# YunjiKim/Unsupervised-Keypoint-Learning-for-Guiding-Class-conditional-Video-Prediction

Hardware: AMD Instinct MI355X
Metric: detector_translator train frames/sec @128x128 K=15 (higher is better)
Workload: dtype f32

## Files before the change

profiles/step_breakdown.py:

```python
#!/usr/bin/env python3
import csv
import sys

FAMILIES = [
    ('bf16-storage 3x3 conv fwd/dgrad (conv3x3_bf16s)', ('conv3x3_bf16s_kernel',)),
    ('bf16 3x3 weight gradient (conv3x3_wgrad_bf16 + slab reduce)', ('conv3x3_wgrad_bf16_kernel', 'wgrad16_reduce_kernel')),
    ('bf16 filter preparation', ('conv_bf16s_prepare',)),
    ('bf16 <-> fp32 conversions / bf16 channel copies', ('cast_channels_kernel',)),
    ('F(4x4,3x3) Winograd fwd/dgrad, bf16x3 form (conv_wino43b)', ('conv_wino43b_kernel',)),
    ('F(4x4,3x3) Winograd fwd/dgrad, fp32 MFMA (conv_wino43)', ('conv_wino43_kernel',)),
    ('F(2x2,3x3) Winograd fwd/dgrad', ('conv_wino_v2_kernel',)),
    ('Winograd weight gradient', ('conv_wino_wgrad_kernel',)),
    ('bf16x3 gather conv fwd/dgrad (conv_gemm3)', ('conv_gemm3_kernel',)),
    ('bf16x3 weight gradient (conv_wgrad3)', ('conv_wgrad3_kernel',)),
    ('fp32-MFMA direct conv fwd/dgrad', ('conv_igemm_kernel', 'conv_small_cout_kernel')),
    ('fp32-MFMA direct weight gradients', ('conv_wgrad_kernel', 'conv_wgrad_rows', 'conv_wgrad_tap_rows', 'conv_wgrad_rows_merged', 'conv_c16_wgrad', 'wgrad_small')),
    ('split-K / weight-gradient slab reductions', ('wgrad_reduce_kernel', 'splitk_reduce_kernel')),
    ('16-cout / image-input conv kernels', ('conv3x3_c16_kernel', 'conv_rgb', 'conv_few')),
    ('batch norm', ('bn_', 'chan_reduce_kernel<1', 'chan_reduce_kernel<2', 'chan_reduce_bf16_kernel<1', 'chan_reduce_bf16_kernel<2')),
    ('bias gradients (channel sums)', ('chan_reduce_kernel<0', 'chan_reduce_bf16_kernel<0', 'chan_sum_finalize')),
    ('Winograd filter transforms', ('filter_transform',)),
    ('key-point head / heat-map render', ('kp_', 'gauss_')),
    ('VGG19 pointwise (prep, pool, feature gradient, L1)', ('vgg_', 'maxpool2', 'l1_pair')),
    ('resize / concat / copy / activation backward / blend', ('resize2x', 'copy_channels', 'act_bwd', 'head_blend', 'fill_kernel', 'axpy')),
    ('Adam', ('adam_tf',)),
    ('losses', ('xent',)),
    ('torch glue (adds, mean)', ('at::native',)),
]


def main():
    path, steps = sys.argv[1], float(sys.argv[2])
    rows = list(csv.DictReader(open(path)))
    fam = {name: [0.0, 0] for name, _ in FAMILIES}
    other = [0.0, 0, []]
    for r in rows:
        ns, calls = float(r['TotalDurationNs']), int(r['Calls'])
        for name, keys in FAMILIES:
            if any(k in r['Name'] for k in keys):
                fam[name][0] += ns; fam[name][1] += calls
                break
        else:
            other[0] += ns; other[1] += calls; other[2].append(r['Name'][:50])
    total = sum(v[0] for v in fam.values()) + other[0]
    launches = sum(v[1] for v in fam.values()) + other[1]
    print('%-58s %9s %10s' % ('kernel family', 'ms/step', 'launches/step'))
    for name, _ in FAMILIES:
        ns, calls = fam[name]
        if calls:
            print('%-58s %9.3f %10.1f' % (name, ns / 1e6 / steps, calls / steps))
    if other[1]:
        print('%-58s %9.3f %10.1f   %s' % ('other', other[0] / 1e6 / steps, other[1] / steps, sorted(set(other[2]))[:6]))
    print('%-58s %9.3f %10.1f   (sum over the three streams)' % ('TOTAL', total / 1e6 / steps, launches / steps))


if __name__ == '__main__':
    main()
```

unsupervised-keypoint-learning-for-guiding-class-conditional-video-prediction_amd/csrc/conv_wino.hip:

```cpp
#include "kpx_internal.h"
#include "kpx_env.h"
#include <stdlib.h>
#include <type_traits>
#include <atomic>

struct WinoGeom {
    const float* x; float* y; const float* U; const float* bias;
    int N, H, W, Cin, ldx, Cout, ldy, act;
    int pack;
    int Kp, Np;
    int tiles_y, tiles_x, nt;
    int stagger;
    float* stats;
    const float* mask_y; int ld_mask;
    const float* bn_beta;
};

static __device__ __attribute__((aligned(16))) float wino_zero16[4] = {0.f, 0.f, 0.f, 0.f};

template <bool DGRAD>
__global__ __launch_bounds__(256) void wino_filter_transform_frag_kernel(const float* __restrict__ w, int Cin, int Cout, int Kp, int Np, float* __restrict__ Uf) {
    const int K = DGRAD ? Cout : Cin, Nn = DGRAD ? Cin : Cout;
    const int KC = Kp >> 3, NB = Np >> 5;
    const size_t total = (size_t)Kp * Np;
    for (size_t idx = (size_t)blockIdx.x * 256 + threadIdx.x; idx < total; idx += (size_t)gridDim.x * 256) {
        const int j = (int)(idx & 3), li = (int)((idx >> 2) & 31), lh = (int)((idx >> 7) & 1);
        const size_t blk = idx >> 8;
        const int nb = (int)(blk % NB), kc = (int)(blk / NB);
        const int c = 8 * kc + 4 * lh + j, n = 32 * nb + li;
        const bool real = c < K && n < Nn;
        float g[3][3];
#pragma unroll
        for (int r = 0; r < 3; ++r)
#pragma unroll
            for (int q = 0; q < 3; ++q)
                g[r][q] = !real ? 0.f : (DGRAD ? w[((size_t)((2 - r) * 3 + (2 - q)) * Cin + n) * Cout + c] : w[((size_t)(r * 3 + q) * Cin + c) * Cout + n]);
        float t[4][3];
#pragma unroll
        for (int q = 0; q < 3; ++q) {
            t[0][q] = g[0][q];
            t[1][q] = 0.5f * (g[0][q] + g[1][q] + g[2][q]);
            t[2][q] = 0.5f * (g[0][q] - g[1][q] + g[2][q]);
            t[3][q] = g[2][q];
        }
        const size_t pstride = (size_t)KC * NB * 256;
        float* o = Uf + blk * 256 + (idx & 255);
#pragma unroll
        for (int i = 0; i < 4; ++i) {
            o[(size_t)(i * 4 + 0) * pstride] = t[i][0];
            o[(size_t)(i * 4 + 1) * pstride] = 0.5f * (t[i][0] + t[i][1] + t[i][2]);
            o[(size_t)(i * 4 + 2) * pstride] = 0.5f * (t[i][0] - t[i][1] + t[i][2]);
            o[(size_t)(i * 4 + 3) * pstride] = t[i][2];
        }
    }
}

__device__ __forceinline__ int w8_pos(int p) { return p < 8 ? p : (p == 16 ? 8 : (p == 17 ? 17 : p + 1)); }
__device__ __forceinline__ int w8_pix(int pos) { return pos < 8 ? pos : (pos == 8 ? 16 : (pos == 17 ? 17 : pos - 1)); }

#define W2_RAW 3200
#define W2_V 8192
#define W2_MAIN (2 * W2_RAW + 2 * W2_V)

#ifdef KPX_WINO_STAMP
__device__ unsigned long long* wino_dbg = nullptr;
extern "C" int kpx_debug_wino_stamps(unsigned long long* buf) { return -(int)hipMemcpyToSymbol(HIP_SYMBOL(wino_dbg), &buf, sizeof(buf)); }
#define W2_STAMP(slot) do { if (dbg) dbg[(slot)] = __builtin_amdgcn_s_memtime(); } while (0)
#else
#define W2_STAMP(slot) do { } while (0)
#endif

template <int MODE, int STATS>
__global__ __launch_bounds__(512, 2) void conv_wino_v2_kernel(const WinoGeom g) {
    extern __shared__ __attribute__((aligned(16))) float smem[];
    constexpr int NC = 32 * MODE, NTG = MODE;
    float* const rawb = smem;
    float* const Vb = smem + 2 * W2_RAW;

    const int t = threadIdx.x, lane = t & 63, wave = t >> 6;
    const int li = lane & 31, lh = lane >> 5;
    const int wa = wave & 3, hsel = wave >> 2;
    int L = kpx_xcd_remap(blockIdx.x, gridDim.x);
    const int ntc = g.Np / NC;
    const int nti = L % ntc; L /= ntc;
    const int bx = L % g.tiles_x; L /= g.tiles_x;
    const int by = L % g.tiles_y;
    const int n = g.pack ? 4 * L : L / g.tiles_y;
    const int oy0 = by * 16, ox0 = bx * 16, n0 = nti * NC;

    const float* rp[2]; bool rok[2];
#pragma unroll
    for (int i = 0; i < 2; ++i) {
        const int u = t + 512 * i, q = u >> 1, py = q / 20, ps = q - py * 20;
        int iy, ix, ni = n;
        bool ok;
        if (g.pack) {
            const int sy = py / 10, sx = ps / 10;
            iy = py - 10 * sy - 1; ix = ps - 10 * sx - 1; ni = n + 2 * sy + sx;
            ok = u < 800 && (unsigned)iy < 8u && (unsigned)ix < 8u;
        } else {
            iy = oy0 - 1 + py; ix = ox0 - 1 + w8_pix(ps);
            ok = u < 720 && ps < 18 && (unsigned)iy < (unsigned)g.H && (unsigned)ix < (unsigned)g.W;
        }
        if (g.Cin <= 4 && (u & 1)) ok = false;
        rok[i] = ok;
        rp[i] = ok ? g.x + ((size_t)(ni * g.H + iy) * g.W + ix) * g.ldx + (u & 1) * 4 : wino_zero16;
    }
    const int KC = g.Kp >> 3, NB = g.Np >> 5;
    const int nb = MODE == 2 ? nti * 2 + hsel : nti;
    const size_t ub_pstride = (size_t)KC * NB * 256, ub_step = (size_t)NB * 256;
    const float* ubp = g.U + ((size_t)(4 * wa) * KC * NB + nb) * 256 + lane * 4;
    const int tslot = t & 1, ttile = (t >> 1) & 63, vrow = t >> 7;
    const int tty = ttile >> 3, ttx = ttile & 7;
    const int ra = vrow == 0 ? 0 : (vrow == 2 ? 2 : 1), rb = vrow == 0 ? 2 : (vrow == 1 ? 2 : (vrow == 2 ? 1 : 3));
    const float sgn = vrow == 1 ? 1.f : -1.f;
    int trd[4];
#pragma unroll
    for (int c = 0; c < 4; ++c)
        trd[c] = g.pack ? ((tty >> 2) * 10 + 2 * (tty & 3) + ra) * 160 + ((ttx >> 2) * 10 + 2 * (ttx & 3) + c) * 8 + tslot * 4
                        : (2 * tty + ra) * 160 + w8_pos(2 * ttx + c) * 8 + tslot * 4;
    const int trb = (rb - ra) * 160;
    const int vwr = (vrow * 4) * 512 + ttile * 8 + ((tslot ^ ((ttile >> 3) & 1)) << 2);
    int a_rd[NTG];
#pragma unroll
    for (int i = 0; i < NTG; ++i) {
        const int tile = (MODE == 2 ? i : hsel) * 32 + li;
        a_rd[i] = (4 * wa) * 512 + tile * 8 + ((lh ^ ((tile >> 3) & 1)) << 2);
    }

    f32x16 acc[4][NTG];
#pragma unroll
    for (int b = 0; b < 4; ++b)
#pragma unroll
        for (int i = 0; i < NTG; ++i)
#pragma unroll
            for (int r = 0; r < 16; ++r) acc[b][i][r] = 0.f;

    const int nchunks = g.Kp / 8;
    const int ktail = g.Cin - (nchunks - 1) * 8 - tslot * 4;
    f32x4 rr[2], ub[4];
    auto load_raw = [&]() {
#pragma unroll
        for (int i = 0; i < 2; ++i) { rr[i] = *reinterpret_cast<const f32x4*>(rp[i]); if (rok[i]) rp[i] += 8; }
    };
    const int st2 = t < 288 ? (t + 512) * 4 : t * 4;
    auto stage = [&](float* rawW) {
        *reinterpret_cast<f32x4*>(&rawW[t * 4]) = rr[0];
        *reinterpret_cast<f32x4*>(&rawW[st2]) = t < 288 ? rr[1] : rr[0];
    };
    auto transform = [&](const float* rawR, float* Vw, bool mask_tail) {
        f32x4 tr[4];
#pragma unroll
        for (int c = 0; c < 4; ++c) {
            const f32x4 a = *reinterpret_cast<const f32x4*>(&rawR[trd[c]]);
            const f32x4 b = *reinterpret_cast<const f32x4*>(&rawR[trd[c] + trb]);
            tr[c] = a + sgn * b;
        }
        if (mask_tail) {
#pragma unroll
            for (int c = 0; c < 4; ++c)
#pragma unroll
                for (int j = 0; j < 4; ++j) if (j >= ktail) tr[c][j] = 0.f;
        }
        *reinterpret_cast<f32x4*>(&Vw[vwr]) = tr[0] - tr[2];
        *reinterpret_cast<f32x4*>(&Vw[vwr + 512]) = tr[1] + tr[2];
        *reinterpret_cast<f32x4*>(&Vw[vwr + 1024]) = tr[2] - tr[1];
        *reinterpret_cast<f32x4*>(&Vw[vwr + 1536]) = tr[1] - tr[3];
    };
    auto mfma = [&](const float* Vr, bool refill) {
        f32x4 av[2][NTG];
#pragma unroll
        for (int i = 0; i < NTG; ++i) av[0][i] = *reinterpret_cast<const f32x4*>(&Vr[a_rd[i]]);
#pragma unroll
        for (int b = 0; b < 4; ++b) {
            if (b < 3) {
#pragma unroll
                for (int i = 0; i < NTG; ++i) av[(b + 1) & 1][i] = *reinterpret_cast<const f32x4*>(&Vr[a_rd[i] + (b + 1) * 512]);
            }
#pragma unroll
            for (int j = 0; j < 4; ++j)
#pragma unroll
                for (int i = 0; i < NTG; ++i)
                    acc[b][i] = __builtin_amdgcn_mfma_f32_32x32x2f32(av[b & 1][i][j], ub[b][j], acc[b][i], 0, 0, 0);
            if (refill) ub[b] = *reinterpret_cast<const f32x4*>(ubp + (size_t)b * ub_pstride);
        }
        ubp += ub_step;
    };
    const bool late = g.stagger && __builtin_amdgcn_readfirstlane(t) >= 256;
#ifdef KPX_WINO_STAMP
    unsigned long long* dbg = (wino_dbg && lane == 0 && (wave & 3) == 0 && blockIdx.x < 64) ? wino_dbg + ((size_t)blockIdx.x * 2 + (wave >> 2)) * 256 : nullptr;
    if (dbg) { dbg[0] = __builtin_amdgcn_s_memtime(); dbg[1] = __builtin_amdgcn_s_memrealtime(); }
#endif
    auto body = [&](int k, auto full_tag, auto parity_tag) {
        constexpr bool FULL = decltype(full_tag)::value;
        constexpr int PAR = decltype(parity_tag)::value;
        const int cur = PAR == 2 ? (k & 1) : PAR;
        float* const rawC = rawb + cur * W2_RAW;
        float* const rawN = rawb + (cur ^ 1) * W2_RAW;
        float* const Vc = Vb + cur * W2_V;
        float* const Vn = Vb + (cur ^ 1) * W2_V;
        W2_STAMP(8 + 4 * k);
        __syncthreads();
        W2_STAMP(9 + 4 * k);
        if (late) mfma(Vc, FULL || k + 1 < nchunks);
        if (late) W2_STAMP(10 + 4 * k);
        if (FULL || k + 1 < nchunks) transform(rawN, Vn, !FULL && k + 1 == nchunks - 1 && ktail < 4);
        if (FULL || k + 2 < nchunks) stage(rawC);
        if (FULL || k + 3 < nchunks) load_raw();
        if (!late) W2_STAMP(10 + 4 * k);
        if (!late) mfma(Vc, FULL || k + 1 < nchunks);
        W2_STAMP(11 + 4 * k);
    };

    load_raw();
#pragma unroll
    for (int b = 0; b < 4; ++b) ub[b] = *reinterpret_cast<const f32x4*>(ubp + (size_t)b * ub_pstride);
    ubp += ub_step;
    stage(rawb);
    if (nchunks > 1) load_raw();
    __syncthreads();
    transform(rawb, Vb, nchunks == 1 && ktail < 4);
    if (nchunks > 1) stage(rawb + W2_RAW);
    if (nchunks > 2) load_raw();
    int k = 0;
    for (; k + 4 < nchunks; k += 2) {
        body(k, std::true_type{}, std::integral_constant<int, 0>{});
        body(k + 1, std::true_type{}, std::integral_constant<int, 1>{});
    }
    for (; k < nchunks; ++k) body(k, std::false_type{}, std::integral_constant<int, 2>{});

#ifdef KPX_WINO_STAMP
    if (dbg) { dbg[2] = __builtin_amdgcn_s_memtime(); }
#endif
    __syncthreads();
    float* const P = smem;
#pragma unroll
    for (int i = 0; i < NTG; ++i) {
        const int tg = MODE == 2 ? i : hsel;
#pragma unroll
        for (int r = 0; r < 16; ++r) {
            const float m0 = acc[0][i][r], m1 = acc[1][i][r], m2 = acc[2][i][r], m3 = acc[3][i][r];
            const int tile = tg * 32 + (r & 3) + 8 * (r >> 2) + 4 * lh;
            const int col = (MODE == 2 ? hsel * 32 : 0) + li;
            P[((wa * 2 + 0) * 64 + tile) * NC + col] = m0 + m1 + m2;
            P[((wa * 2 + 1) * 64 + tile) * NC + col] = m1 - m2 - m3;
        }
    }
    const bool mask_vec = STATS == 2 && (g.ld_mask & 3) == 0 && ((reinterpret_cast<uintptr_t>(g.mask_y) & 15) == 0);
    f32x4 ym[MODE][4];
    if (STATS == 2) {
#pragma unroll
        for (int it = 0; it < MODE; ++it) {
            const int idx = t + 512 * it;
            const int tile = idx / (NC / 4), cq = idx - tile * (NC / 4), c0 = n0 + cq * 4;
            const int oy = oy0 + 2 * (tile >> 3), ox = ox0 + 2 * (tile & 7);
#pragma unroll
            for (int px = 0; px < 4; ++px) {
                const float* my = g.mask_y + ((size_t)(n * g.H + oy + (px >> 1)) * g.W + ox + (px & 1)) * g.ld_mask + c0;
                ym[it][px] = f32x4{0.f, 0.f, 0.f, 0.f};
                if (mask_vec && c0 + 3 < g.Cout) ym[it][px] = *reinterpret_cast<const f32x4*>(my);
                else {
#pragma unroll
                    for (int e = 0; e < 4; ++e) if (c0 + e < g.Cout) ym[it][px][e] = my[e];
                }
            }
        }
    }
    __syncthreads();
    const bool vec_ok = (g.ldy & 3) == 0 && ((reinterpret_cast<uintptr_t>(g.y) & 15) == 0);
    f32x4 st_s = {0.f, 0.f, 0.f, 0.f}, st_q = {0.f, 0.f, 0.f, 0.f};
#pragma unroll
    for (int it = 0; it < MODE; ++it) {
        const int idx = t + 512 * it;
        const int tile = idx / (NC / 4), cq = idx - tile * (NC / 4);
        f32x4 pv[4][2];
#pragma unroll
        for (int a = 0; a < 4; ++a)
#pragma unroll
            for (int j = 0; j < 2; ++j) pv[a][j] = *reinterpret_cast<const f32x4*>(&P[((a * 2 + j) * 64 + tile) * NC + cq * 4]);
        const int c0 = n0 + cq * 4;
        f32x4 bv = {0.f, 0.f, 0.f, 0.f};
        if (g.bias) {
#pragma unroll
            for (int e = 0; e < 4; ++e) if (c0 + e < g.Cout) bv[e] = g.bias[c0 + e];
        }
        f32x4 bvec = {0.f, 0.f, 0.f, 0.f};
        if (STATS == 2) {
#pragma unroll
            for (int e = 0; e < 4; ++e) if (c0 + e < g.Cout) bvec[e] = g.bn_beta[c0 + e];
        }
        const int ty = tile >> 3, tx = tile & 7;
        const int on = g.pack ? n + 2 * (ty >> 2) + (tx >> 2) : n;
        const int oy = g.pack ? 2 * (ty & 3) : oy0 + 2 * ty, ox = g.pack ? 2 * (tx & 3) : ox0 + 2 * tx;
#pragma unroll
        for (int dy = 0; dy < 2; ++dy)
#pragma unroll
            for (int dx = 0; dx < 2; ++dx) {
                f32x4 v = (dy == 0 ? pv[0][dx] + pv[1][dx] + pv[2][dx] : pv[1][dx] - pv[2][dx] - pv[3][dx]) + bv;
                if (g.act == KPX_ACT_RELU) {
#pragma unroll
                    for (int e = 0; e < 4; ++e) v[e] = fmaxf(v[e], 0.f);
                } else if (g.act == KPX_ACT_LRELU) {
#pragma unroll
                    for (int e = 0; e < 4; ++e) v[e] = v[e] > 0.f ? v[e] : 0.01f * v[e];
                }
                if (STATS == 2) {
                    const f32x4 yv = ym[it][dy * 2 + dx];
#pragma unroll
                    for (int e = 0; e < 4; ++e) {
                        const float dz = yv[e] > 0.f ? v[e] : 0.f;
                        st_s[e] += dz; st_q[e] += dz * (yv[e] - bvec[e]);
                    }
                } else if (STATS == 1) { st_s += v; st_q += v * v; }
                float* o = g.y + ((size_t)(on * g.H + oy + dy) * g.W + ox + dx) * g.ldy + c0;
                if (vec_ok && c0 + 3 < g.Cout) *reinterpret_cast<f32x4*>(o) = v;
                else {
#pragma unroll
                    for (int e = 0; e < 4; ++e) if (c0 + e < g.Cout) o[e] = v[e];
                }
            }
    }
    if (STATS != 0) {
        __syncthreads();
        float* const S = smem;
        *reinterpret_cast<f32x4*>(&S[t * 8]) = st_s;
        *reinterpret_cast<f32x4*>(&S[t * 8 + 4]) = st_q;
        __syncthreads();
        if (t < 2 * NC) {
            const int stat = t / NC, c = t - stat * NC, cq = c >> 2, e = c & 3;
            float r = 0.f;
#pragma unroll 8
            for (int m = 0; m < 512 / (NC / 4); ++m) r += S[(cq + (NC / 4) * m) * 8 + stat * 4 + e];
            const size_t tile_id = ((size_t)n * g.tiles_y + by) * g.tiles_x + bx;
            if (n0 + c < g.Cout) g.stats[(tile_id * 2 + stat) * g.Cout + n0 + c] = r;
        }
    }
#ifdef KPX_WINO_STAMP
    if (dbg) { dbg[3] = __builtin_amdgcn_s_memtime(); dbg[4] = __builtin_amdgcn_s_memrealtime(); }
#endif
}

static inline int w2_lds_bytes(int mode) { const int main = W2_MAIN * 4, epi = 4 * 2 * 64 * 32 * mode * 4; return main > epi ? main : epi; }

static std::atomic<unsigned long long> wino_attr_mask{0};

extern "C" int kpx_conv3x3_wino_eligible(int N, int H, int W, int K, int Nn, int ldin, const void* in_ptr) {
    if (kpx_env()->no_wino || N <= 0 || K <= 0 || Nn <= 0) return 0;
    const bool shape = (H % 16 == 0 && W % 16 == 0) || (H == 8 && W == 8 && N % 4 == 0);
    const int kmin = 4, nmin = 4;
    const bool kfit = ldin >= ((K + 7) & ~7) || K == 4;
    return shape && K >= kmin && Nn >= nmin && (K >= 16 || K == 4 || K == 8) && kfit && (ldin % 4 == 0) && (((uintptr_t)in_ptr) & 15) == 0;
}
extern "C" __attribute__((visibility("hidden"))) int kpx_wino_eligible(int N, int H, int W, int K, int Nn, int ldin, const void* in_ptr) {
    return kpx_conv3x3_wino_eligible(N, H, W, K, Nn, ldin, in_ptr);
}

extern "C" size_t kpx_wino_u_bytes(int Cin, int Cout) {
    const size_t a = (size_t)((Cin + 7) & ~7) * ((Cout + 31) & ~31), b = (size_t)((Cout + 7) & ~7) * ((Cin + 31) & ~31);
    return 16 * 4 * (a > b ? a : b);
}

extern "C" int kpx_wino_filter_transform_f32(const float* w_hwio, int Cin, int Cout, int dgrad, float* U, void* stream) {
    if (!w_hwio || !U || Cin <= 0 || Cout <= 0) return KPX_EINVAL;
    const int K = dgrad ? Cout : Cin, Nn = dgrad ? Cin : Cout;
    const int Kp = (K + 7) & ~7, Np = (Nn + 31) & ~31;
    const size_t pairs = (size_t)Kp * Np;
    size_t nb = (pairs + 255) / 256; if (nb > 1024) nb = 1024;
    hipStream_t s = kpx_stream(stream);
    if (dgrad) hipLaunchKernelGGL(wino_filter_transform_frag_kernel<true>, dim3((unsigned)nb), dim3(256), 0, s, w_hwio, Cin, Cout, Kp, Np, U);
    else hipLaunchKernelGGL(wino_filter_transform_frag_kernel<false>, dim3((unsigned)nb), dim3(256), 0, s, w_hwio, Cin, Cout, Kp, Np, U);
    return kpx_launch_status();
}

__global__ __launch_bounds__(256) void wino_filter_transform_batch_kernel(const KpxWinoDesc* __restrict__ descs) {
    const KpxWinoDesc d = descs[blockIdx.y];
    const int Cin = d.cin, Cout = d.cout;
    const bool dg = d.dgrad != 0;
    const int K = dg ? Cout : Cin, Nn = dg ? Cin : Cout;
    const int Kp = (K + 7) & ~7, Np = (Nn + 31) & ~31, KC = Kp >> 3, NB = Np >> 5;
    const size_t total = (size_t)Kp * Np, pstride = (size_t)KC * NB * 256;
    const float* __restrict__ w = d.w;
    float* __restrict__ Uf = d.u;
    for (size_t idx = (size_t)blockIdx.x * 256 + threadIdx.x; idx < total; idx += (size_t)gridDim.x * 256) {
        const int j = (int)(idx & 3), li = (int)((idx >> 2) & 31), lh = (int)((idx >> 7) & 1);
        const size_t blk = idx >> 8;
        const int nb = (int)(blk % NB), kc = (int)(blk / NB);
        const int c = 8 * kc + 4 * lh + j, n = 32 * nb + li;
        const bool real = c < K && n < Nn;
        float g[3][3];
#pragma unroll
        for (int r = 0; r < 3; ++r)
#pragma unroll
            for (int q = 0; q < 3; ++q)
                g[r][q] = !real ? 0.f : (dg ? w[((size_t)((2 - r) * 3 + (2 - q)) * Cin + n) * Cout + c] : w[((size_t)(r * 3 + q) * Cin + c) * Cout + n]);
        float t[4][3];
#pragma unroll
        for (int q = 0; q < 3; ++q) {
            t[0][q] = g[0][q];
            t[1][q] = 0.5f * (g[0][q] + g[1][q] + g[2][q]);
            t[2][q] = 0.5f * (g[0][q] - g[1][q] + g[2][q]);
            t[3][q] = g[2][q];
        }
        float* o = Uf + blk * 256 + (idx & 255);
#pragma unroll
        for (int i = 0; i < 4; ++i) {
            o[(size_t)(i * 4 + 0) * pstride] = t[i][0];
            o[(size_t)(i * 4 + 1) * pstride] = 0.5f * (t[i][0] + t[i][1] + t[i][2]);
            o[(size_t)(i * 4 + 2) * pstride] = 0.5f * (t[i][0] - t[i][1] + t[i][2]);
            o[(size_t)(i * 4 + 3) * pstride] = t[i][2];
        }
    }
}
extern "C" int kpx_wino_filter_transform_batch_f32(const void* descs_dev, int n, void* stream) {
    if (!descs_dev || n <= 0 || n > 65535) return KPX_EINVAL;
    hipLaunchKernelGGL(wino_filter_transform_batch_kernel, dim3(64, (unsigned)n), dim3(256), 0, kpx_stream(stream), (const KpxWinoDesc*)descs_dev);
    return kpx_launch_status();
}

extern "C" size_t kpx_conv3x3_wino_stats_tiles(int N, int H, int W) {
    return (H % 16 || W % 16 || N <= 0) ? 0 : (size_t)N * (H / 16) * (W / 16);
}
static int wino_launch(const float* in, int N, int H, int W, int K, int ldin, const float* U, const float* bias,
                       float* out, int Nn, int ldout, int act, float* tile_stats, void* stream,
                       const float* mask_y, int ld_mask, const float* bn_beta) {
    if (!in || !U || !out || ldin < (K == 4 ? 4 : K) || ldout < Nn || act < 0 || act > 2 || !kpx_conv3x3_wino_eligible(N, H, W, K, Nn, ldin, in)) return KPX_EINVAL;
    hipStream_t s = kpx_stream(stream);
    if (kpx_first_use_on_device(&wino_attr_mask)) {
        hipError_t e = hipSuccess;
#define W2_ATTR(M, S) if (e == hipSuccess) e = hipFuncSetAttribute(reinterpret_cast<const void*>(conv_wino_v2_kernel<M, S>), hipFuncAttributeMaxDynamicSharedMemorySize, w2_lds_bytes(M))
        W2_ATTR(1, 0); W2_ATTR(2, 0); W2_ATTR(1, 1); W2_ATTR(2, 1); W2_ATTR(1, 2); W2_ATTR(2, 2);
#undef W2_ATTR
        if (e != hipSuccess) return -(int)e;
    }
    WinoGeom g{};
    g.x = in; g.y = out; g.U = U; g.bias = bias; g.stats = tile_stats;
    g.mask_y = mask_y; g.ld_mask = ld_mask; g.bn_beta = bn_beta;
    g.N = N; g.H = H; g.W = W; g.Cin = K; g.ldx = ldin; g.Cout = Nn; g.ldy = ldout; g.act = act;
    g.Kp = (K + 7) & ~7; g.Np = (Nn + 31) & ~31;
    g.pack = (H == 8 && W == 8) ? 1 : 0;
    g.tiles_y = g.pack ? 1 : H / 16; g.tiles_x = g.pack ? 1 : W / 16; g.nt = g.Np / 32;
    const unsigned blocks = (unsigned)((size_t)(g.pack ? N / 4 : N) * g.tiles_y * g.tiles_x * g.nt);
    const bool wide = blocks / 2 >= 256 && g.Np % 64 == 0;
    g.stagger = 1;
    const int st = !tile_stats ? 0 : (mask_y ? 2 : 1);
#define W2_GO(M, S) hipLaunchKernelGGL((conv_wino_v2_kernel<M, S>), dim3(M == 2 ? blocks / 2 : blocks), dim3(512), w2_lds_bytes(M), s, g)
    if (wide) { if (st == 0) W2_GO(2, 0); else if (st == 1) W2_GO(2, 1); else W2_GO(2, 2); }
    else { if (st == 0) W2_GO(1, 0); else if (st == 1) W2_GO(1, 1); else W2_GO(1, 2); }
#undef W2_GO
    return kpx_launch_status();
}

extern "C" int kpx_conv3x3_wino_f32(const float* in, int N, int H, int W, int K, int ldin, const float* U, const float* bias,
                                    float* out, int Nn, int ldout, int act, float* tile_stats, const float* bn_y, int ld_bn_y,
                                    const float* bn_beta, void* stream) {
    if (tile_stats && (H % 16 || W % 16)) return KPX_EINVAL;
    if ((bn_y || bn_beta) && (!tile_stats || !bn_y || !bn_beta || ld_bn_y < Nn || bias || act != KPX_ACT_NONE)) return KPX_EINVAL;
    return wino_launch(in, N, H, W, K, ldin, U, bias, out, Nn, ldout, act, tile_stats, stream, bn_y, ld_bn_y, bn_beta);
}

extern "C" __attribute__((visibility("hidden"))) int kpx_wino_conv3x3(const float* in, int N, int H, int W, int K, int ldin, const float* w_hwio, int Cin, int Cout, int dgrad,
                                const float* bias, int act, float* out, int Nn, int ldout, float* U_ws, hipStream_t s) {
    int rc = kpx_wino_filter_transform_f32(w_hwio, Cin, Cout, dgrad, U_ws, (void*)s);
    if (rc) return rc;
    return kpx_conv3x3_wino_f32(in, N, H, W, K, ldin, U_ws, bias, out, Nn, ldout, act, nullptr, nullptr, 0, nullptr, (void*)s);
}

struct WinoWgradGeom {
    const float* x; const float* dy; float* out;
    int N, H, W, Cin, ldx, Cout, lddy;
    int cit, cot, S, cps, total_chunks, chy, chx;
    size_t slab;
};

template <int CIT, int COT>
__global__ __launch_bounds__(512, 2) void conv_wino_wgrad_kernel(const WinoWgradGeom g) {
    constexpr int CI = 32 * CIT, CO = 32 * COT, SI = CI / 4, SO = CO / 4;
    constexpr int VF = 16 * 8 * CI, DF = 16 * 8 * CO, BUF = VF + DF;
    extern __shared__ __attribute__((aligned(16))) float smem[];

    const int t = threadIdx.x, lane = t & 63, wave = __builtin_amdgcn_readfirstlane(t >> 6), li = lane & 31, lh = lane >> 5;
    int L = kpx_xcd_remap(blockIdx.x, gridDim.x);
    const int split = L % g.S; L /= g.S;
    const int cot = L % g.cot, cit = L / g.cot;
    const int c0 = cit * CI, n0 = cot * CO;

    const int vsl = (t % SI) * 4, vtile = (t / SI) & 7, vrow = t / (8 * SI);
    const int esl = (t % SO) * 4, etile = (t / SO) & 7, erow = t / (8 * SO);
    const bool vthr = t < 32 * SI, ethr = t < 32 * SO;
    const bool vact = vthr && c0 + vsl < g.Cin, eact = ethr && n0 + esl < g.Cout;
    const int xtail = g.Cin - (c0 + vsl);
    const int ra = vrow == 0 ? 0 : (vrow == 2 ? 2 : 1), rb = vrow == 0 ? 2 : (vrow == 1 ? 2 : (vrow == 2 ? 1 : 3));
    const float sgn = vrow == 1 ? 1.f : -1.f;
    const int pya = 2 * (vtile >> 2) + ra - 1, pyb = 2 * (vtile >> 2) + rb - 1, px0 = 2 * (vtile & 3) - 1;
    const int vwr = (vrow * 4) * 8 * CI + vtile * CI + vsl;
    const float d0 = erow == 3 ? 0.f : 1.f, d1 = erow == 0 ? 0.f : (erow == 1 ? 1.f : -1.f);
    const int dwr = VF + (erow * 4) * 8 * CO + etile * CO + esl;
    const int dyo = ((2 * (etile >> 2) * g.W + 2 * (etile & 3)) * g.lddy + n0 + esl) * 4;
    const int OOB = (int)0x80000000;
    const __amdgpu_buffer_rsrc_t rsx = __builtin_amdgcn_make_buffer_rsrc(const_cast<float*>(g.x) - (size_t)(g.W + 1) * g.ldx, 0, 0x7fffffff, 0x00020000);
    const __amdgpu_buffer_rsrc_t rsd = __builtin_amdgcn_make_buffer_rsrc(const_cast<float*>(g.dy), 0, 0x7fffffff, 0x00020000);
    int vxa[4], vxb[4], vd[4];
#pragma unroll
    for (int c = 0; c < 4; ++c) {
        vxa[c] = vact ? (((pya + 1) * g.W + px0 + c + 1) * g.ldx + c0 + vsl) * 4 : OOB;
        vxb[c] = vact ? (((pyb + 1) * g.W + px0 + c + 1) * g.ldx + c0 + vsl) * 4 : OOB;
    }
    vd[0] = eact ? dyo : OOB; vd[1] = eact ? dyo + g.lddy * 4 : OOB; vd[2] = eact ? dyo + g.W * g.lddy * 4 : OOB; vd[3] = eact ? dyo + (g.W + 1) * g.lddy * 4 : OOB;
    const bool top_a = pya < 0, bot_a = pya > 3, top_b = pyb < 0, bot_b = pyb > 3, left0 = px0 < 0, right3 = px0 + 3 > 7;
    const int p0 = 2 * wave;

    f32x16 acc[2][CIT][COT];
#pragma unroll
    for (int a = 0; a < 2; ++a)
#pragma unroll
        for (int b = 0; b < CIT; ++b)
#pragma unroll
            for (int c = 0; c < COT; ++c)
#pragma unroll
                for (int r = 0; r < 16; ++r) acc[a][b][c][r] = 0.f;

    const int ch_begin = split * g.cps;
    int ch_end = ch_begin + g.cps; if (ch_end > g.total_chunks) ch_end = g.total_chunks;
    const int nch = ch_end - ch_begin;
    const int lq = ch_begin / g.chx;
    int lcx = __builtin_amdgcn_readfirstlane(ch_begin - lq * g.chx);
    int lcy = __builtin_amdgcn_readfirstlane(lq % g.chy), ln = __builtin_amdgcn_readfirstlane(lq / g.chy);
    f32x4 rxa[4], rxb[4], rd[4];
    auto load_next = [&]() {
        const int pix = (ln * g.H + lcy * 4) * g.W + lcx * 8;
        const int sx = pix * g.ldx * 4, sd = pix * g.lddy * 4;
        const bool s_top = lcy == 0, s_bot = lcy + 1 == g.chy, s_left = lcx == 0, s_right = lcx + 1 == g.chx;
        const bool inv_a = (top_a && s_top) || (bot_a && s_bot), inv_b = (top_b && s_top) || (bot_b && s_bot);
#pragma unroll
        for (int c = 0; c < 4; ++c) {
            const bool inv_c = (c == 0 && left0 && s_left) || (c == 3 && right3 && s_right);
            rxa[c] = __builtin_bit_cast(f32x4, __builtin_amdgcn_raw_buffer_load_b128(rsx, (inv_a || inv_c) ? OOB : vxa[c], sx, 0));
            rxb[c] = __builtin_bit_cast(f32x4, __builtin_amdgcn_raw_buffer_load_b128(rsx, (inv_b || inv_c) ? OOB : vxb[c], sx, 0));
        }
#pragma unroll
        for (int i = 0; i < 4; ++i) rd[i] = __builtin_bit_cast(f32x4, __builtin_amdgcn_raw_buffer_load_b128(rsd, vd[i], sd, 0));
        if (++lcx == g.chx) { lcx = 0; if (++lcy == g.chy) { lcy = 0; ++ln; } }
    };
    auto transform = [&](float* buf) {
        if (vthr) {
            f32x4 tr[4];
#pragma unroll
            for (int c = 0; c < 4; ++c) tr[c] = rxa[c] + sgn * rxb[c];
            if (g.Cin & 3) {
#pragma unroll
                for (int c = 0; c < 4; ++c)
#pragma unroll
                    for (int j = 1; j < 4; ++j) if (j >= xtail) tr[c][j] = 0.f;
            }
            *reinterpret_cast<f32x4*>(&buf[vwr]) = tr[0] - tr[2];
            *reinterpret_cast<f32x4*>(&buf[vwr + 8 * CI]) = tr[1] + tr[2];
            *reinterpret_cast<f32x4*>(&buf[vwr + 16 * CI]) = tr[2] - tr[1];
            *reinterpret_cast<f32x4*>(&buf[vwr + 24 * CI]) = tr[1] - tr[3];
        }
        if (ethr) {
            const f32x4 t0 = d0 * rd[0] + d1 * rd[2], t1 = d0 * rd[1] + d1 * rd[3];
            *reinterpret_cast<f32x4*>(&buf[dwr]) = t0;
            *reinterpret_cast<f32x4*>(&buf[dwr + 8 * CO]) = t0 + t1;
            *reinterpret_cast<f32x4*>(&buf[dwr + 16 * CO]) = t0 - t1;
            *reinterpret_cast<f32x4*>(&buf[dwr + 24 * CO]) = -t1;
        }
    };
    auto mfma = [&](const float* buf) {
#pragma unroll
        for (int pt = 0; pt < 2; ++pt) {
            const float* Vp = buf + (p0 + pt) * 8 * CI + lh * CI + li;
            const float* Dp = buf + VF + (p0 + pt) * 8 * CO + lh * CO + li;
#pragma unroll
            for (int s = 0; s < 4; ++s) {
                float a[CIT], b[COT];
#pragma unroll
                for (int i = 0; i < CIT; ++i) a[i] = Vp[s * 2 * CI + i * 32];
#pragma unroll
                for (int j = 0; j < COT; ++j) b[j] = Dp[s * 2 * CO + j * 32];
#pragma unroll
                for (int i = 0; i < CIT; ++i)
#pragma unroll
                    for (int j = 0; j < COT; ++j)
                        acc[pt][i][j] = __builtin_amdgcn_mfma_f32_32x32x2f32(a[i], b[j], acc[pt][i][j], 0, 0, 0);
            }
        }
    };
    const bool late = wave >= 4;
    if (nch > 0) {
        load_next();
        transform(smem);
        if (nch > 1) load_next();
    }
    for (int k = 0; k < nch; ++k) {
        float* const cur = smem + (k & 1) * BUF;
        float* const nxt = smem + ((k & 1) ^ 1) * BUF;
        __syncthreads();
        if (late) mfma(cur);
        if (k + 1 < nch) transform(nxt);
        if (k + 2 < nch) load_next();
        if (!late) mfma(cur);
    }
    __syncthreads();

    float* Ms = smem;
    float* out = g.out + (size_t)split * g.slab;
    const int oc = t & 31;
#pragma unroll
    for (int q = 0; q < CIT * COT; ++q) {
        const int ci = q / COT, co = q % COT;
        if (q) __syncthreads();
#pragma unroll
        for (int pt = 0; pt < 2; ++pt)
#pragma unroll
            for (int r = 0; r < 16; ++r)
                Ms[((p0 + pt) * 32 + (r & 3) + 8 * (r >> 2) + 4 * lh) * 32 + li] = acc[pt][ci][co][r];
        __syncthreads();
#pragma unroll
        for (int i = 0; i < 2; ++i) {
            const int cl = (t >> 5) + 16 * i;
            float m[16];
#pragma unroll
            for (int p = 0; p < 16; ++p) m[p] = Ms[(p * 32 + cl) * 32 + oc];
            float h[3][4];
#pragma unroll
            for (int j = 0; j < 4; ++j) {
                h[0][j] = m[j] + 0.5f * (m[4 + j] + m[8 + j]);
                h[1][j] = 0.5f * (m[4 + j] - m[8 + j]);
                h[2][j] = 0.5f * (m[4 + j] + m[8 + j]) + m[12 + j];
            }
            const int c = c0 + ci * 32 + cl, n = n0 + co * 32 + oc;
            if (c < g.Cin && n < g.Cout) {
                float* o = out + (size_t)c * g.Cout + n;
                const size_t tap = (size_t)g.Cin * g.Cout;
#pragma unroll
                for (int r = 0; r < 3; ++r) {
                    o[(r * 3 + 0) * tap] = h[r][0] + 0.5f * (h[r][1] + h[r][2]);
                    o[(r * 3 + 1) * tap] = 0.5f * (h[r][1] - h[r][2]);
                    o[(r * 3 + 2) * tap] = 0.5f * (h[r][1] + h[r][2]) + h[r][3];
                }
            }
        }
    }
}

static inline int ww_tile(int C) { return (C % 64 == 0 || C > 96) ? 2 : 1; }

extern "C" __attribute__((visibility("hidden"))) int kpx_wino_wgrad_splits(int N, int H, int W, int Cin, int Cout) {
    if (kpx_env()->no_wino) return 0;
    const int comin = 4;
    if (H % 4 || W % 8 || Cout % 4 || Cin < 32 || Cout < comin) return 0;
    const int ti = ww_tile(Cin), to = ww_tile(Cout);
    if (ti == 1 && to == 1) return 0;
    const long tc = (long)N * (H / 4) * (W / 8), tiles = (long)((Cin + 32 * ti - 1) / (32 * ti)) * ((Cout + 32 * to - 1) / (32 * to));
    const long target = 256;
    long S = target / tiles;
    if (S < 1) S = 1;
    if (S > tc / 8) S = tc / 8;
    const long cap = (128L << 20) / ((long)9 * Cin * Cout * 4);
    if (S > cap) S = cap;
    if (S < 1) S = 1;
    if (tc < 64 || tiles * S < 128) return 0;
    return (int)S;
}

extern "C" __attribute__((visibility("hidden"))) int kpx_wino_wgrad3x3(const float* x, int N, int H, int W, int Cin, int ldx, const float* dy, int Cout, int lddy,
                                                                   float* slabs, int S, hipStream_t s) {
    static std::atomic<unsigned long long> attr_mask{0};
    const int lds22 = 2 * (16 * 8 * 64 + 16 * 8 * 64) * 4, lds21 = 2 * (16 * 8 * 64 + 16 * 8 * 32) * 4, lds12 = 2 * (16 * 8 * 32 + 16 * 8 * 64) * 4;
    if (kpx_first_use_on_device(&attr_mask)) {
        hipError_t e = hipFuncSetAttribute(reinterpret_cast<const void*>(conv_wino_wgrad_kernel<2, 2>), hipFuncAttributeMaxDynamicSharedMemorySize, lds22);
        if (e == hipSuccess) e = hipFuncSetAttribute(reinterpret_cast<const void*>(conv_wino_wgrad_kernel<2, 1>), hipFuncAttributeMaxDynamicSharedMemorySize, lds21 > 65536 ? lds21 : 65536);
        if (e == hipSuccess) e = hipFuncSetAttribute(reinterpret_cast<const void*>(conv_wino_wgrad_kernel<1, 2>), hipFuncAttributeMaxDynamicSharedMemorySize, lds12 > 65536 ? lds12 : 65536);
        if (e != hipSuccess) return -(int)e;
    }
    const int ti = ww_tile(Cin), to = ww_tile(Cout);
    WinoWgradGeom g{};
    g.x = x; g.dy = dy; g.out = slabs;
    g.N = N; g.H = H; g.W = W; g.Cin = Cin; g.ldx = ldx; g.Cout = Cout; g.lddy = lddy;
    g.cit = (Cin + 32 * ti - 1) / (32 * ti); g.cot = (Cout + 32 * to - 1) / (32 * to); g.S = S;
    g.chy = H / 4; g.chx = W / 8; g.total_chunks = N * g.chy * g.chx;
    g.cps = (g.total_chunks + S - 1) / S;
    g.slab = (size_t)9 * Cin * Cout;
    const dim3 grid((unsigned)(g.cit * g.cot * S));
    if (ti == 2 && to == 2) hipLaunchKernelGGL((conv_wino_wgrad_kernel<2, 2>), grid, dim3(512), lds22, s, g);
    else if (ti == 2) hipLaunchKernelGGL((conv_wino_wgrad_kernel<2, 1>), grid, dim3(512), lds21 > 65536 ? lds21 : 65536, s, g);
    else hipLaunchKernelGGL((conv_wino_wgrad_kernel<1, 2>), grid, dim3(512), lds12 > 65536 ? lds12 : 65536, s, g);
    return kpx_launch_status();
}
```

unsupervised-keypoint-learning-for-guiding-class-conditional-video-prediction_amd/csrc/kpx_env.h:

```cpp
#pragma once

struct KpxEnv {
    int no_wino;
    int no_gemm3;
    int bf16s_variant;
};

extern "C" __attribute__((visibility("hidden"))) const KpxEnv* kpx_env();
```

unsupervised-keypoint-learning-for-guiding-class-conditional-video-prediction_amd/csrc/kpx_env.hip:

```cpp
#include <stdio.h>
#include <stdlib.h>
#include <atomic>
#include <mutex>
#include "kpx_env.h"
#include "../../include/kpx.h"

static KpxEnv g_env;
static std::atomic<int> g_env_loaded{0};
static std::mutex g_env_mutex;

static int env_flag(const char* name) { return getenv(name) != nullptr; }
static long env_long(const char* name, long dflt) { const char* v = getenv(name); return v ? atol(v) : dflt; }

static void env_parse(KpxEnv* e) {
    e->no_wino = env_flag("KPX_NO_WINO");
    e->no_gemm3 = env_flag("KPX_NO_GEMM3");
    e->bf16s_variant = (int)env_long("KPX_BF16S_VARIANT", 0);
}

extern "C" __attribute__((visibility("hidden"))) const KpxEnv* kpx_env() {
    if (!g_env_loaded.load(std::memory_order_acquire)) {
        std::lock_guard<std::mutex> lock(g_env_mutex);
        if (!g_env_loaded.load(std::memory_order_relaxed)) {
            env_parse(&g_env);
            g_env_loaded.store(1, std::memory_order_release);
        }
    }
    return &g_env;
}

extern "C" int kpx_reload_env(void) {
    std::lock_guard<std::mutex> lock(g_env_mutex);
    env_parse(&g_env);
    g_env_loaded.store(1, std::memory_order_release);
    return 0;
}
```

unsupervised-keypoint-learning-for-guiding-class-conditional-video-prediction_amd/csrc/kpx_internal.h:

```cpp
#pragma once
#include "conv_geom.h"

static inline bool kpx_offsets_fit(size_t pixels, size_t ld, size_t limit) { return pixels * ld * 4 < limit; }

extern "C" __attribute__((visibility("hidden"))) int kpx_gemm3_eligible(const ConvGeom* g);
extern "C" __attribute__((visibility("hidden"))) int kpx_gemm3_launch(ConvGeom g, int bt, int terms, hipStream_t s);
extern "C" __attribute__((visibility("hidden"))) int kpx_wgrad3_eligible(const WgradGeom* g);
extern "C" __attribute__((visibility("hidden"))) int kpx_wgrad3_launch(WgradGeom g, int bm, int terms, hipStream_t s);

extern "C" __attribute__((visibility("hidden"))) int kpx_wino_eligible(int N, int H, int W, int K, int Nn, int ldin, const void* in_ptr);
extern "C" __attribute__((visibility("hidden"))) int kpx_wino_conv3x3(const float* in, int N, int H, int W, int K, int ldin, const float* w_hwio, int Cin, int Cout, int dgrad,
                                const float* bias, int act, float* out, int Nn, int ldout, float* U_ws, hipStream_t s);
extern "C" __attribute__((visibility("hidden"))) int kpx_wino_wgrad_splits(int N, int H, int W, int Cin, int Cout);
extern "C" __attribute__((visibility("hidden"))) int kpx_wino_wgrad3x3(const float* x, int N, int H, int W, int Cin, int ldx, const float* dy, int Cout, int lddy,
                                 float* slabs, int S, hipStream_t s);

extern "C" __attribute__((visibility("hidden"))) int kpx_conv_rgb_fwd(const float* x, int N, int Hi, int Wi, int Cin, const float* w, int KH, int KW,
                                const float* bias, float* y, int Ho, int Wo, int Cout, int ldy,
                                int stride, int pad_t, int pad_l, int act, hipStream_t s, int y16 = 0);
extern "C" __attribute__((visibility("hidden"))) int kpx_conv_rgb_dgrad(const float* dy, int N, int Ho, int Wo, int Cout, int lddy, const float* w, int KH, int KW,
                                  float* dx, int Hi, int Wi, int Cin, int lddx, int stride, int pad_t, int pad_l, hipStream_t s, int dy16 = 0);
extern "C" __attribute__((visibility("hidden"))) int kpx_conv_few_fwd(const float* x, int N, int Hi, int Wi, int Cin, int ldx, const float* w, int KH, int KW,
                                const float* bias, float* y, int Ho, int Wo, int Cout, int ldy,
                                int stride, int pad_t, int pad_l, int act, hipStream_t s);

extern "C" __attribute__((visibility("hidden"))) int kpx_wsmall_splits(int N, int Hi, int Wi, int Cin, int Ho, int Wo, int Cout, int KH, int KW, int stride);
extern "C" __attribute__((visibility("hidden"))) int kpx_wsmall_launch(const float* x, int N, int Hi, int Wi, int Cin, int ldx, const float* dy, int Ho, int Wo, int Cout, int lddy,
                                 int KH, int KW, int stride, int pad_t, int pad_l, float* slabs, int S, hipStream_t s, int dy16 = 0);
```

Baseline: 1399.

## Add bf16x3 Winograd weight-gradient kernel with row-split slabs and LDS transpose reads

Adds a new Winograd weight-gradient kernel that splits fp32 transformed inputs into three bf16 terms and accumulates with 32x32x16 bf16 MFMA, reading fragments with ds_read_tr16 transposes. Each slab handles one of four Winograd rows, so the transform work is split across blocks. Loads are double-buffered so that half the waves run MFMA while the other half transform the next chunk. It is dispatched when channels are multiples of 64 and the split count is a multiple of 4, with an env flag to disable it. In exchange it writes full 9-tap slabs per row (many of them zero), which adds reduce traffic, and it risks small precision differences.

```diff
diff --git a/profiles/step_breakdown.py b/profiles/step_breakdown.py
--- a/profiles/step_breakdown.py
+++ b/profiles/step_breakdown.py
@@ -10,7 +10,7 @@
     ('F(4x4,3x3) Winograd fwd/dgrad, bf16x3 form (conv_wino43b)', ('conv_wino43b_kernel',)),
     ('F(4x4,3x3) Winograd fwd/dgrad, fp32 MFMA (conv_wino43)', ('conv_wino43_kernel',)),
     ('F(2x2,3x3) Winograd fwd/dgrad', ('conv_wino_v2_kernel',)),
-    ('Winograd weight gradient', ('conv_wino_wgrad_kernel',)),
+    ('Winograd weight gradient', ('conv_wino_wgrad_kernel', 'conv_wino_wgrad3_kernel')),
     ('bf16x3 gather conv fwd/dgrad (conv_gemm3)', ('conv_gemm3_kernel',)),
     ('bf16x3 weight gradient (conv_wgrad3)', ('conv_wgrad3_kernel',)),
     ('fp32-MFMA direct conv fwd/dgrad', ('conv_igemm_kernel', 'conv_small_cout_kernel')),
diff --git a/unsupervised-keypoint-learning-for-guiding-class-conditional-video-prediction_amd/csrc/conv_wino.hip b/unsupervised-keypoint-learning-for-guiding-class-conditional-video-prediction_amd/csrc/conv_wino.hip
--- a/unsupervised-keypoint-learning-for-guiding-class-conditional-video-prediction_amd/csrc/conv_wino.hip
+++ b/unsupervised-keypoint-learning-for-guiding-class-conditional-video-prediction_amd/csrc/conv_wino.hip
@@ -666,6 +666,8 @@
 extern "C" __attribute__((visibility("hidden"))) int kpx_wino_wgrad3x3(const float* x, int N, int H, int W, int Cin, int ldx, const float* dy, int Cout, int lddy,
                                                                    float* slabs, int S, hipStream_t s) {
     static std::atomic<unsigned long long> attr_mask{0};
+    if (!kpx_env()->no_wino_wgrad3 && Cin % 64 == 0 && Cout % 64 == 0 && S >= 4 && S % 4 == 0)
+        return kpx_wino_wgrad3_launch(x, N, H, W, Cin, ldx, dy, Cout, lddy, slabs, S, s);
     const int lds22 = 2 * (16 * 8 * 64 + 16 * 8 * 64) * 4, lds21 = 2 * (16 * 8 * 64 + 16 * 8 * 32) * 4, lds12 = 2 * (16 * 8 * 32 + 16 * 8 * 64) * 4;
     if (kpx_first_use_on_device(&attr_mask)) {
         hipError_t e = hipFuncSetAttribute(reinterpret_cast<const void*>(conv_wino_wgrad_kernel<2, 2>), hipFuncAttributeMaxDynamicSharedMemorySize, lds22);
diff --git a/unsupervised-keypoint-learning-for-guiding-class-conditional-video-prediction_amd/csrc/conv_wino_wgrad3.hip b/unsupervised-keypoint-learning-for-guiding-class-conditional-video-prediction_amd/csrc/conv_wino_wgrad3.hip
--- /dev/null
+++ b/unsupervised-keypoint-learning-for-guiding-class-conditional-video-prediction_amd/csrc/conv_wino_wgrad3.hip
@@ -0,0 +1,218 @@
+#include "kpx_internal.h"
+#include "kpx_bf16.h"
+
+struct WinoWgrad3Geom {
+    const float* x; const float* dy; float* out;
+    int N, H, W, Cin, ldx, Cout, lddy;
+    int cit, cot, S, cps, total_chunks, chy, chx;
+    size_t slab;
+};
+
+typedef short s16x4 __attribute__((ext_vector_type(4)));
+typedef __attribute__((address_space(3))) s16x4* lds_s16x4_ptr;
+
+#define WW3_IMG 2048
+#define WW3_SIDE (12 * WW3_IMG)
+#define WW3_BUF (2 * WW3_SIDE)
+#define WW3_LDS (2 * WW3_BUF)
+
+__global__ __launch_bounds__(512, 2) void conv_wino_wgrad3_kernel(const WinoWgrad3Geom g) {
+    extern __shared__ __attribute__((aligned(16))) unsigned char smem3[];
+
+    const int t = threadIdx.x, lane = t & 63, wave = __builtin_amdgcn_readfirstlane(t >> 6), li = lane & 31, lh = lane >> 5;
+    int L = kpx_xcd_remap(blockIdx.x, gridDim.x);
+    const int slab_id = L % g.S; L /= g.S;
+    const int cot = L % g.cot, cit = L / g.cot;
+    const int row = slab_id & 3, split = slab_id >> 2;
+    const int c0 = cit * 64, n0 = cot * 64;
+
+    const bool xside = wave < 4;
+    const int half = (wave >> 1) & 1;
+    const int slot = t & 15, tile = (t >> 4) & 15, tile8 = tile & 7;
+    const int ra = row == 0 ? 0 : (row == 2 ? 2 : 1), rb = row == 0 ? 2 : (row == 1 ? 2 : (row == 2 ? 1 : 3));
+    const float sgn = row == 1 ? 1.f : -1.f;
+    const float d0 = row == 3 ? 0.f : 1.f, d1 = row == 0 ? 0.f : (row == 1 ? 1.f : -1.f);
+    const int pya = 2 * (tile8 >> 2) + ra - 1, pyb = 2 * (tile8 >> 2) + rb - 1, px0 = 2 * (tile8 & 3) - 1;
+    const int iwr = (xside ? 0 : WW3_SIDE) + tile * 128 + ((slot * 8) ^ (((tile >> 1) & 1) << 6));
+    const int OOB = (int)0x80000000;
+    const __amdgpu_buffer_rsrc_t rsx = __builtin_amdgcn_make_buffer_rsrc(const_cast<float*>(g.x) - (size_t)(g.W + 1) * g.ldx, 0, 0x7fffffff, 0x00020000);
+    const __amdgpu_buffer_rsrc_t rsd = __builtin_amdgcn_make_buffer_rsrc(const_cast<float*>(g.dy), 0, 0x7fffffff, 0x00020000);
+    int vo[8];
+    if (xside) {
+#pragma unroll
+        for (int c = 0; c < 4; ++c) {
+            vo[c] = (((pya + 1) * g.W + px0 + c + 1) * g.ldx + c0 + slot * 4) * 4;
+            vo[4 + c] = (((pyb + 1) * g.W + px0 + c + 1) * g.ldx + c0 + slot * 4) * 4;
+        }
+    } else {
+        const int dyo = ((2 * (tile8 >> 2) * g.W + 2 * (tile8 & 3)) * g.lddy + n0 + slot * 4) * 4;
+        vo[0] = dyo; vo[1] = dyo + g.lddy * 4; vo[2] = dyo + g.W * g.lddy * 4; vo[3] = dyo + (g.W + 1) * g.lddy * 4;
+#pragma unroll
+        for (int c = 4; c < 8; ++c) vo[c] = OOB;
+    }
+    const bool top_a = pya < 0, bot_a = pya > 3, top_b = pyb < 0, bot_b = pyb > 3, left0 = px0 < 0, right3 = px0 + 3 > 7;
+
+    const int col = wave & 3, ci = wave >> 2;
+    f32x16 acc[2], lo[2];
+#pragma unroll
+    for (int j = 0; j < 2; ++j)
+#pragma unroll
+        for (int r = 0; r < 16; ++r) acc[j][r] = lo[j][r] = 0.f;
+    const int rq = (lane >> 2) & 3, rp = lane & 3, gq = lane >> 4;
+    const int rd_lane = (8 * lh + rq) * 128 + (((16 * (gq & 1) + 4 * rp) * 2) ^ (((rq >> 1) & 1) << 6));
+    const int a_rd = (col * WW3_IMG + rd_lane) ^ (ci << 6);
+    const int b_rd = WW3_SIDE + col * WW3_IMG + rd_lane;
+
+    const int ch_begin = split * g.cps;
+    int ch_end = ch_begin + g.cps; if (ch_end > g.total_chunks) ch_end = g.total_chunks;
+    const int nch = ch_end - ch_begin;
+    const int nst = nch > 0 ? (nch + 1) >> 1 : 0;
+    int lch = __builtin_amdgcn_readfirstlane(ch_begin + half);
+    const int lq = lch / g.chx;
+    int lcx = __builtin_amdgcn_readfirstlane(lch - lq * g.chx);
+    int lcy = __builtin_amdgcn_readfirstlane(lq % g.chy), ln = __builtin_amdgcn_readfirstlane(lq / g.chy);
+    f32x4 r0[8];
+    auto load_next = [&](f32x4 (&rr)[8]) {
+        const bool past = lch >= ch_end;
+        const int pix = past ? 0 : (ln * g.H + lcy * 4) * g.W + lcx * 8;
+        const bool s_top = lcy == 0, s_bot = lcy + 1 == g.chy, s_left = lcx == 0, s_right = lcx + 1 == g.chx;
+        if (xside) {
+            const int sx = pix * g.ldx * 4;
+            const bool inv_a = past || (top_a && s_top) || (bot_a && s_bot), inv_b = past || (top_b && s_top) || (bot_b && s_bot);
+#pragma unroll
+            for (int c = 0; c < 4; ++c) {
+                const bool inv_c = (c == 0 && left0 && s_left) || (c == 3 && right3 && s_right);
+                rr[c] = __builtin_bit_cast(f32x4, __builtin_amdgcn_raw_buffer_load_b128(rsx, (inv_a || inv_c) ? OOB : vo[c], sx, 0));
+                rr[4 + c] = __builtin_bit_cast(f32x4, __builtin_amdgcn_raw_buffer_load_b128(rsx, (inv_b || inv_c) ? OOB : vo[4 + c], sx, 0));
+            }
+        } else {
+            const int sd = pix * g.lddy * 4;
+#pragma unroll
+            for (int i = 0; i < 4; ++i) rr[i] = __builtin_bit_cast(f32x4, __builtin_amdgcn_raw_buffer_load_b128(rsd, past ? OOB : vo[i], sd, 0));
+        }
+        lch += 2;
+#pragma unroll
+        for (int i = 0; i < 2; ++i)
+            if (++lcx == g.chx) { lcx = 0; if (++lcy == g.chy) { lcy = 0; ++ln; } }
+    };
+    auto put = [&](unsigned char* img, const f32x4 v) {
+        unsigned lo[3], hi[3];
+        kpx_split2<3>(v[0], v[1], lo);
+        kpx_split2<3>(v[2], v[3], hi);
+#pragma unroll
+        for (int tm = 0; tm < 3; ++tm) *reinterpret_cast<u32x2*>(img + tm * 4 * WW3_IMG) = u32x2{lo[tm], hi[tm]};
+    };
+    auto transform = [&](unsigned char* buf, const f32x4 (&rr)[8]) {
+        unsigned char* const w = buf + iwr;
+        if (xside) {
+            f32x4 tr[4];
+#pragma unroll
+            for (int c = 0; c < 4; ++c) tr[c] = rr[c] + sgn * rr[4 + c];
+            put(w, tr[0] - tr[2]);
+            put(w + WW3_IMG, tr[1] + tr[2]);
+            put(w + 2 * WW3_IMG, tr[2] - tr[1]);
+            put(w + 3 * WW3_IMG, tr[1] - tr[3]);
+        } else {
+            const f32x4 t0 = d0 * rr[0] + d1 * rr[2], t1 = d0 * rr[1] + d1 * rr[3];
+            put(w, t0);
+            put(w + WW3_IMG, t0 + t1);
+            put(w + 2 * WW3_IMG, t0 - t1);
+            put(w + 3 * WW3_IMG, -t1);
+        }
+    };
+    auto frag = [&](const unsigned char* p) {
+        const u32x2 v0 = __builtin_bit_cast(u32x2, __builtin_amdgcn_ds_read_tr16_b64_v4i16((lds_s16x4_ptr)(p)));
+        const u32x2 v1 = __builtin_bit_cast(u32x2, __builtin_amdgcn_ds_read_tr16_b64_v4i16((lds_s16x4_ptr)(p + 512)));
+        return __builtin_bit_cast(bf16x8, u32x4{v0[0], v0[1], v1[0], v1[1]});
+    };
+    auto mfma = [&](const unsigned char* buf) {
+        bf16x8 a[3], b[2][3];
+#pragma unroll
+        for (int tm = 0; tm < 3; ++tm) {
+            a[tm] = frag(buf + a_rd + tm * 4 * WW3_IMG);
+            b[0][tm] = frag(buf + b_rd + tm * 4 * WW3_IMG);
+            b[1][tm] = frag(buf + (b_rd ^ 64) + tm * 4 * WW3_IMG);
+        }
+#pragma unroll
+        for (int j = 0; j < 2; ++j) {
+            f32x16 c = lo[j];
+            c = __builtin_amdgcn_mfma_f32_32x32x16_bf16(a[2], b[j][0], c, 0, 0, 0);
+            c = __builtin_amdgcn_mfma_f32_32x32x16_bf16(a[0], b[j][2], c, 0, 0, 0);
+            c = __builtin_amdgcn_mfma_f32_32x32x16_bf16(a[1], b[j][1], c, 0, 0, 0);
+            c = __builtin_amdgcn_mfma_f32_32x32x16_bf16(a[1], b[j][0], c, 0, 0, 0);
+            lo[j] = __builtin_amdgcn_mfma_f32_32x32x16_bf16(a[0], b[j][1], c, 0, 0, 0);
+            acc[j] = __builtin_amdgcn_mfma_f32_32x32x16_bf16(a[0], b[j][0], acc[j], 0, 0, 0);
+        }
+    };
+    const bool late = wave >= 4;
+    if (nst > 0) {
+        load_next(r0);
+        transform(smem3, r0);
+        if (nst > 1) load_next(r0);
+    }
+    auto iter = [&](int k, auto parity) {
+        constexpr int P = decltype(parity)::value;
+        unsigned char* const cur = smem3 + P * WW3_BUF;
+        unsigned char* const nxt = smem3 + (P ^ 1) * WW3_BUF;
+        __syncthreads();
+        if (late) mfma(cur);
+        if (k + 1 < nst) transform(nxt, r0);
+        if (k + 2 < nst) load_next(r0);
+        if (!late) mfma(cur);
+    };
+    for (int k = 0; k < nst; k += 2) {
+        iter(k, kpx_ic<0>{});
+        if (k + 1 < nst) iter(k + 1, kpx_ic<1>{});
+    }
+    __syncthreads();
+
+    float* Ms = reinterpret_cast<float*>(smem3);
+#pragma unroll
+    for (int j = 0; j < 2; ++j)
+#pragma unroll
+        for (int r = 0; r < 16; ++r)
+            Ms[(col * 64 + ci * 32 + (r & 3) + 8 * (r >> 2) + 4 * lh) * 64 + j * 32 + li] = acc[j][r] + lo[j][r];
+    __syncthreads();
+    const float gw0 = row == 0 ? 1.f : (row == 3 ? 0.f : 0.5f), gw1 = row == 1 ? 0.5f : (row == 2 ? -0.5f : 0.f), gw2 = row == 3 ? 1.f : (row == 0 ? 0.f : 0.5f);
+    float* out = g.out + (size_t)slab_id * g.slab;
+    const size_t tap = (size_t)g.Cin * g.Cout;
+    const int oc = t & 63;
+#pragma unroll
+    for (int i = 0; i < 8; ++i) {
+        const int cl = (t >> 6) + 8 * i;
+        float m[4];
+#pragma unroll
+        for (int p = 0; p < 4; ++p) m[p] = Ms[(p * 64 + cl) * 64 + oc];
+        float h[3];
+        h[0] = m[0] + 0.5f * (m[1] + m[2]);
+        h[1] = 0.5f * (m[1] - m[2]);
+        h[2] = 0.5f * (m[1] + m[2]) + m[3];
+        float* o = out + (size_t)(c0 + cl) * g.Cout + n0 + oc;
+#pragma unroll
+        for (int q = 0; q < 3; ++q) {
+            o[(0 * 3 + q) * tap] = gw0 == 0.f ? 0.f : gw0 * h[q];
+            o[(1 * 3 + q) * tap] = gw1 == 0.f ? 0.f : gw1 * h[q];
+            o[(2 * 3 + q) * tap] = gw2 == 0.f ? 0.f : gw2 * h[q];
+        }
+    }
+}
+
+extern "C" __attribute__((visibility("hidden"))) int kpx_wino_wgrad3_launch(const float* x, int N, int H, int W, int Cin, int ldx, const float* dy, int Cout, int lddy,
+                                                                        float* slabs, int S, hipStream_t s) {
+    static std::atomic<unsigned long long> attr_mask{0};
+    if (Cin % 64 || Cout % 64 || S < 4 || S % 4 || H % 4 || W % 8) return KPX_EINVAL;
+    if (kpx_first_use_on_device(&attr_mask)) {
+        hipError_t e = hipFuncSetAttribute(reinterpret_cast<const void*>(conv_wino_wgrad3_kernel), hipFuncAttributeMaxDynamicSharedMemorySize, WW3_LDS);
+        if (e != hipSuccess) return -(int)e;
+    }
+    WinoWgrad3Geom g{};
+    g.x = x; g.dy = dy; g.out = slabs;
+    g.N = N; g.H = H; g.W = W; g.Cin = Cin; g.ldx = ldx; g.Cout = Cout; g.lddy = lddy;
+    g.cit = Cin / 64; g.cot = Cout / 64; g.S = S;
+    g.chy = H / 4; g.chx = W / 8; g.total_chunks = N * g.chy * g.chx;
+    const int ps = S / 4;
+    g.cps = (g.total_chunks + ps - 1) / ps;
+    g.slab = (size_t)9 * Cin * Cout;
+    hipLaunchKernelGGL(conv_wino_wgrad3_kernel, dim3((unsigned)(g.cit * g.cot * S)), dim3(512), WW3_LDS, s, g);
+    return kpx_launch_status();
+}
diff --git a/unsupervised-keypoint-learning-for-guiding-class-conditional-video-prediction_amd/csrc/kpx_env.h b/unsupervised-keypoint-learning-for-guiding-class-conditional-video-prediction_amd/csrc/kpx_env.h
--- a/unsupervised-keypoint-learning-for-guiding-class-conditional-video-prediction_amd/csrc/kpx_env.h
+++ b/unsupervised-keypoint-learning-for-guiding-class-conditional-video-prediction_amd/csrc/kpx_env.h
@@ -3,6 +3,7 @@
 struct KpxEnv {
     int no_wino;
     int no_gemm3;
+    int no_wino_wgrad3;
     int bf16s_variant;
 };
 
diff --git a/unsupervised-keypoint-learning-for-guiding-class-conditional-video-prediction_amd/csrc/kpx_env.hip b/unsupervised-keypoint-learning-for-guiding-class-conditional-video-prediction_amd/csrc/kpx_env.hip
--- a/unsupervised-keypoint-learning-for-guiding-class-conditional-video-prediction_amd/csrc/kpx_env.hip
+++ b/unsupervised-keypoint-learning-for-guiding-class-conditional-video-prediction_amd/csrc/kpx_env.hip
@@ -15,6 +15,7 @@
 static void env_parse(KpxEnv* e) {
     e->no_wino = env_flag("KPX_NO_WINO");
     e->no_gemm3 = env_flag("KPX_NO_GEMM3");
+    e->no_wino_wgrad3 = env_flag("KPX_NO_WINO_WGRAD3");
     e->bf16s_variant = (int)env_long("KPX_BF16S_VARIANT", 0);
 }
 
diff --git a/unsupervised-keypoint-learning-for-guiding-class-conditional-video-prediction_amd/csrc/kpx_internal.h b/unsupervised-keypoint-learning-for-guiding-class-conditional-video-prediction_amd/csrc/kpx_internal.h
--- a/unsupervised-keypoint-learning-for-guiding-class-conditional-video-prediction_amd/csrc/kpx_internal.h
+++ b/unsupervised-keypoint-learning-for-guiding-class-conditional-video-prediction_amd/csrc/kpx_internal.h
@@ -14,6 +14,8 @@
 extern "C" __attribute__((visibility("hidden"))) int kpx_wino_wgrad_splits(int N, int H, int W, int Cin, int Cout);
 extern "C" __attribute__((visibility("hidden"))) int kpx_wino_wgrad3x3(const float* x, int N, int H, int W, int Cin, int ldx, const float* dy, int Cout, int lddy,
                                  float* slabs, int S, hipStream_t s);
+extern "C" __attribute__((visibility("hidden"))) int kpx_wino_wgrad3_launch(const float* x, int N, int H, int W, int Cin, int ldx, const float* dy, int Cout, int lddy,
+                                      float* slabs, int S, hipStream_t s);
 
 extern "C" __attribute__((visibility("hidden"))) int kpx_conv_rgb_fwd(const float* x, int N, int Hi, int Wi, int Cin, const float* w, int KH, int KW,
                                 const float* bias, float* y, int Ho, int Wo, int Cout, int ldy,
```

New measurement: 1362. 2.6% lower.
